# junejunejune/c_orb_slam

Hardware: AMD Instinct MI355X
Metric: tracking FPS + ORB matches/sec, KITTI-00 stereo; local-BA iter/sec (higher is better)
Workload: dtype u8

## Files before the change

### c_orb_slam_amd/_lib.py

```python
import ctypes as C
import os
import re
from pathlib import Path

import numpy as np

PKG = Path(__file__).resolve().parent
ROOT = PKG.parent
LIB_PATH = Path(os.environ["ORBGPU_LIB"]) if os.environ.get("ORBGPU_LIB") else PKG / "liborbslam_gpu.so"
HEADER = ROOT / "include" / "orbslam_gpu.h"

ORB_OK, ORB_E_INVALID, ORB_E_HIP, ORB_E_CAPACITY, ORB_E_NODEVICE = 0, -1, -2, -3, -4
_ERR = {ORB_E_INVALID: "ORB_E_INVALID", ORB_E_HIP: "ORB_E_HIP", ORB_E_CAPACITY: "ORB_E_CAPACITY",
        ORB_E_NODEVICE: "ORB_E_NODEVICE"}

KP_DTYPE = np.dtype([("x", "<f4"), ("y", "<f4"), ("size", "<f4"), ("angle", "<f4"),
                     ("response", "<f4"), ("octave", "<i4"), ("class_id", "<i4")])
assert KP_DTYPE.itemsize == 28


class OrbGpuError(RuntimeError):
    def __init__(self, code, what=""):
        super().__init__(f"{what}: {_ERR.get(code, code)}")
        self.code = code
# ... 181 lines not shown
    L.Optimizer_last_trace.argtypes = [vp, vp, i32, P(i32), vp, vp, i32, P(i32)]
    L.Optimizer_last_timings.argtypes = [vp]
    L.Optimizer_PoseOptimization.argtypes = [P(pose_problem), vp, vp, P(i32)]
    L.Optimizer_PoseOptimization_batch.argtypes = [i32, vp, vp, vp, vp]
    L.Optimizer_PoseOptimization_batch_device.argtypes = [i32, vp, vp, vp, vp]
    L.Optimizer_OptimizeSim3.argtypes = [vp, vp, vp, P(i32)]
    L.Optimizer_OptimizeSim3_batch.argtypes = [i32, vp, vp, vp, vp]
    L.Optimizer_OptimizeEssentialGraph.argtypes = [vp, i32, vp]
    L.Optimizer_PoseOptimization_frames_device.argtypes = [i32, vp, vp, vp, vp]
    L.Optimizer_pose_timing.argtypes = [i32, vp]
    L.orbgpu_unit_ba_struct.argtypes = [i32, i32, i32, vp, vp, vp, vp, vp, vp, i32, vp, C.c_longlong]
    L.Frame_UnprojectStereo_batch_device.argtypes = [vp, i32, vp]
    L.Frame_UndistortKeyPoints.argtypes = [vp, vp]
    L.Frame_UndistortKeyPoints_batch.argtypes = [vp, i32, vp]
    L.Frame_ComputeImageBounds.argtypes = [vp, i32, i32, vp, vp, i32, vp]
    L.Frame_ComputeStereoFromRGBD.argtypes = [vp, vp, vp]
    L.Frame_ComputeStereoFromRGBD_batch.argtypes = [vp, i32, vp, vp]
    L.ORBvocabulary_create.argtypes = [P(vp)]
    L.ORBvocabulary_destroy.argtypes = [vp]
    L.ORBvocabulary_loadFromTextFile.argtypes = [vp, C.c_char_p]
    L.ORBvocabulary_info.argtypes = [vp, vp, vp, vp, vp, vp, vp]
    L.ORBvocabulary_transform.argtypes = [vp, vp, i32, i32, vp]
    L.ORBvocabulary_transform_batch.argtypes = [vp, i32, vp, vp, i32, vp]
    L.ORBvocabulary_transform_features.argtypes = [vp, vp, i32, i32, vp, vp, vp]
    L.ORBvocabulary_score.argtypes = [vp, vp, vp, i32, i32, vp, vp, vp, vp]
    L.orbgpu_unit_ldlt_solve.argtypes = [i32, vp, vp, vp, i32, P(i32)]
    L.orbgpu_unit_csum.argtypes = [vp, i32, vp]
    L.orbgpu_unit_pnp_layout.argtypes = [i32, vp, vp, vp, vp]
    L.MapPoint_CreateStereo_batch_device.argtypes = [vp, i32, vp]
    L.Tracking_PrepareLocalSearch_batch_device.argtypes = [vp, i32, vp]
    L.ORBmatcher_SearchDense_batch.argtypes = [vp, i32, vp, vp, vp, vp, vp, vp, vp]
    L.ORBmatcher_last_dense_timing.argtypes = [vp, vp, vp]
    L.ORBmatcher_SearchLocalPoints_batch.argtypes = [vp, i32, vp, vp, vp, f32, f32, f32, vp, vp]
    L.Frame_isInFrustum_batch.argtypes = [vp, i32, vp, vp, f32, f32, vp, vp, vp, vp, vp, vp, vp]
    L.ORBmatcher_enable_timing.argtypes = [vp, i32]
    L.ORBmatcher_last_timings.argtypes = [vp, vp, vp]
    L.ORBmatcher_last_search_plan.argtypes = [vp, vp]
    L.orbgpu_unit_ldlt_factor.argtypes = [i32, vp, vp]
    L.orbgpu_unit_wave_tree.argtypes = [vp, vp]
    L.orbgpu_unit_shared_div.argtypes = [vp, vp, i32, vp]
    L.orbgpu_unit_set_csum_lds_max.argtypes = [i32]
    L.orbgpu_unit_set_scale_small_max.argtypes = [i32]
    L.orbgpu_unit_set_struct_gpu_min_edges.argtypes = [i32]
    L.orbgpu_unit_set_posegraph_check.argtypes = [i32]
    L.orbgpu_unit_ba_struct_all.argtypes = [i32, i32, i32, vp, vp, vp, vp, vp, vp, i32, i32, vp, C.c_longlong, vp]
    L.orbgpu_unit_nd_order.argtypes = [i32, vp, vp, i32, vp, vp, vp]
    L.orbgpu_unit_sim3.argtypes = [i32, i32, vp, vp, vp, vp]
    L.orbgpu_unit_essgraph_stage.argtypes = [vp, C.c_double, vp]
    L.orbgpu_unit_set_ess_dense_max.argtypes = [i32]
    L.orbgpu_debug_prof.argtypes = [vp]
    L.orbgpu_debug_prof_match.argtypes = [vp]
    L.orbgpu_debug_prof_extract.argtypes = [vp]
    L.orbgpu_debug_extract_plan.argtypes = [vp, vp, vp, vp]
    L.KeyFrameDatabase_create.argtypes = [vp, P(vp)]
    L.KeyFrameDatabase_destroy.argtypes = [vp]
    L.KeyFrameDatabase_add.argtypes = [vp, C.c_int32, vp, vp, i32]
    L.KeyFrameDatabase_add_batch.argtypes = [vp, i32, vp, vp, vp, vp]
    L.KeyFrameDatabase_erase.argtypes = [vp, C.c_int32]
    L.KeyFrameDatabase_clear.argtypes = [vp]
    L.KeyFrameDatabase_size.argtypes = [vp, P(i32), P(C.c_longlong)]
    L.KeyFrameDatabase_set_covisibles.argtypes = [vp, C.c_int32, i32, vp]
    L.KeyFrameDatabase_DetectLoopCandidates.argtypes = [vp, vp, vp]
    L.KeyFrameDatabase_DetectRelocalizationCandidates.argtypes = [vp, vp, vp]
    L.KeyFrameDatabase_DetectRelocalizationCandidates_batch.argtypes = [vp, i32, vp, vp]
    L.KeyFrameDatabase_enable_timing.argtypes = [vp, i32]
    L.KeyFrameDatabase_last_timings.argtypes = [vp, vp]
    L.orbgpu_unit_set_kfdb_initial_capacity.argtypes = [i32, i32]
    L.Map_create.argtypes = [P(vp)]
    L.Map_destroy.argtypes = [vp]
    L.Map_clear.argtypes = [vp]
    L.Map_size.argtypes = [vp, P(i32), P(C.c_longlong), P(C.c_longlong)]
    L.Map_AddKeyFrame.argtypes = [vp, C.c_int32, i32, vp, vp]
    L.Map_SetMapPointMatches.argtypes = [vp, C.c_int32, i32, vp, vp, vp]
    L.Map_EraseMapPoint.argtypes = [vp, C.c_int32]
    L.Map_ReplaceMapPoint.argtypes = [vp, C.c_int32, C.c_int32]
    L.Map_EraseKeyFrame.argtypes = [vp, C.c_int32]
    L.Map_SetNeighbours.argtypes = [vp, C.c_int32, i32, vp, C.c_int32, i32, vp]
    L.KeyFrame_UpdateConnections.argtypes = [vp, C.c_int32, vp]
    L.KeyFrame_UpdateConnections_batch.argtypes = [vp, i32, vp, vp]
    L.Tracking_UpdateLocalMap_batch.argtypes = [vp, vp, i32, vp]
    L.Map_enable_timing.argtypes = [vp, i32]
    L.Map_last_timings.argtypes = [vp, vp]
    L.orbgpu_unit_set_map_initial_capacity.argtypes = [i32, i32, i32]
    L.orbgpu_unit_set_map_chunk.argtypes = [i32]
    L.orbgpu_unit_set_map_lds_slots.argtypes = [i32]
    L.Initializer_create.argtypes = [vp, i32, vp, f32, i32, P(vp)]
    L.Initializer_destroy.argtypes = [vp]
    L.Initializer_Initialize.argtypes = [vp, i32, vp, vp, vp, vp, vp, vp, vp, P(i32), vp]
    L.Initializer_enable_timing.argtypes = [vp, i32]
    L.Initializer_last_timings.argtypes = [vp, vp]
    L.Sim3Solver_create.argtypes = [i32, vp, vp, vp, vp, vp, i32, vp, vp, i32, P(vp)]
    L.Sim3Solver_destroy.argtypes = [vp]
    L.Sim3Solver_set_ransac.argtypes = [vp, C.c_double, i32, i32]
    L.Sim3Solver_iterate.argtypes = [vp, i32, vp, P(i32), vp, P(i32), vp, P(i32)]
    L.Sim3Solver_iterate_batch.argtypes = [i32, vp, i32, vp, vp, vp, vp, vp, vp]
    L.Sim3Solver_get_estimate.argtypes = [vp, vp, vp, vp]
    L.Sim3Solver_get_state.argtypes = [vp, P(i32), P(i32), P(i32)]
    L.Sim3Solver_enable_timing.argtypes = [i32]
    L.Sim3Solver_last_timings.argtypes = [vp, vp]
    _lib = L
    return L


class orb_rng(C.Structure):
    _fields_ = [("tbl", C.c_int32 * 31), ("f", C.c_int32), ("r", C.c_int32)]

# ... 117 lines not shown
```

### c_orb_slam_amd/csrc/capi_extract.cpp

```cpp
#include <new>

#include "capi_handles.hpp"

extern "C" {

int orbgpu_device_available(void) {
    int n = 0;
    if (hipGetDeviceCount(&n) != hipSuccess) return 0;
    return n > 0 ? 1 : 0;
}

const char* orbgpu_version(void) { return "c_orb_slam_amd 0.2 (gfx950)"; }
int orbgpu_abi_version(void) { return ORBGPU_ABI_VERSION; }

int ORBextractor_create(int nfeatures, float scaleFactor, int nlevels, int iniThFAST, int minThFAST,
                        int max_width, int max_height, int max_batch, ORBextractor_h* out) {
    if (!out || nfeatures < 0 || nlevels < 1 || nlevels > 15 || scaleFactor <= 1.0f || max_width <= 0 ||
        max_height <= 0 || max_batch <= 0 || max_batch > 2047)
        return ORB_E_INVALID;
    *out = nullptr;
    auto* ex = new (std::nothrow) orbgpu::Extractor(nfeatures, scaleFactor, nlevels, iniThFAST, minThFAST);
    if (!ex) return ORB_E_INVALID;
    int rc = ex->init_device(max_width, max_height, max_batch);
    if (rc) {
// ... 63 lines not shown
    return rc == 0 ? ORB_OK : (rc == -2 ? ORB_E_HIP : ORB_E_INVALID);
}

int ORBextractor_get_levels(ORBextractor_h h, int* nlevels, float* scaleFactor) {
    if (!h) return ORB_E_INVALID;
    if (nlevels) *nlevels = h->ex->nlevels();
    if (scaleFactor) *scaleFactor = h->ex->scale_factor();
    return ORB_OK;
}

int ORBextractor_get_scale_tables(ORBextractor_h h, float* scale, float* invScale, float* sigma2, float* invSigma2,
                                  int* nFeaturesPerLevel) {
    if (!h) return ORB_E_INVALID;
    const auto* ex = h->ex;
    for (int l = 0; l < ex->nlevels(); l++) {
        if (scale) scale[l] = ex->scale()[l];
        if (invScale) invScale[l] = ex->inv_scale()[l];
        if (sigma2) sigma2[l] = ex->sigma2()[l];
        if (invSigma2) invSigma2[l] = ex->inv_sigma2()[l];
        if (nFeaturesPerLevel) nFeaturesPerLevel[l] = ex->n_per_level()[l];
    }
    return ORB_OK;
}

void* ORBextractor_stream(ORBextractor_h h) { return h ? (void*)h->ex->stream() : nullptr; }

int ORBextractor_reserve_cus(ORBextractor_h h, int one_in_n) {
    if (!h || one_in_n < 0 || one_in_n == 1) return ORB_E_INVALID;
    const int r = h->ex->reserve_cus(one_in_n);
    return r == -4 ? ORB_E_NODEVICE : r == -1 ? ORB_E_INVALID : (r ? ORB_E_HIP : ORB_OK);
}

int ORBextractor_share_stream(ORBextractor_h h, ORBextractor_h with) {
    if (!h || !with) return ORB_E_INVALID;
    const int r = h->ex->share_stream(with->ex);
    return r == -4 ? ORB_E_NODEVICE : (r ? ORB_E_HIP : ORB_OK);
}

int ORBextractor_last_timings(ORBextractor_h h, float* ms6) {
    if (!h || !ms6) return ORB_E_INVALID;
    return h->ex->timings(ms6);
}

int ORBextractor_last_corner_count(ORBextractor_h h, long long* total) {
    if (!h || !total) return ORB_E_INVALID;
    return h->ex->corner_total(total) ? ORB_E_INVALID : ORB_OK;
}

int orbgpu_debug_extract_plan(ORBextractor_h h, int* flags, int* chain_from, int* tile_rows) {
    if (!h) return ORB_E_INVALID;
    return h->ex->last_plan(flags, chain_from, tile_rows) ? ORB_E_INVALID : ORB_OK;
}

}
```

### c_orb_slam_amd/csrc/orb_extract.hip

```cpp
#include "orb_extract.hpp"

#include <algorithm>
#include <atomic>
#include <chrono>
#include <cmath>
#include <cstring>
#include <thread>

namespace orbgpu {

__constant__ int8_t c_pattern[256 * 4];
__constant__ int8_t c_disc[2 * 1024];
__constant__ int c_ndisc;
__constant__ int c_umax[16];
__constant__ int c_gauss[7];

static const int8_t kPattern[256 * 4] = {
#include "brief_pattern.inc"
};

__device__ __forceinline__ int xcd_tile(int bid, int nb) { return (bid & 7) * (nb >> 3) + (bid >> 3); }
static inline unsigned grid8(int n) { return (unsigned)((n + 7) & ~7); }
constexpr int kFastSplitLevel = 3;

// ... 4 lines not shown
    uint4 o;
    if (x0 >= 0 && x0 + 15 < W) {
        const uintptr_t a = (uintptr_t)(srow + x0);
        const uint32_t* a32 = reinterpret_cast<const uint32_t*>(a & ~(uintptr_t)3);
        const uint32_t sh = (uint32_t)(a & 3);
        const uint32_t w0 = a32[0], w1 = a32[1], w2 = a32[2], w3 = a32[3];
        const uint32_t w4 = sh ? a32[4] : 0u;
        o.x = __builtin_amdgcn_alignbyte(w1, w0, sh);
        o.y = __builtin_amdgcn_alignbyte(w2, w1, sh);
        o.z = __builtin_amdgcn_alignbyte(w3, w2, sh);
        o.w = __builtin_amdgcn_alignbyte(w4, w3, sh);
    } else {
        uint32_t v[4] = {0, 0, 0, 0};
#pragma unroll
        for (int k = 0; k < 16; k++) v[k >> 2] |= (uint32_t)srow[refl101(x0 + k, W)] << (8 * (k & 3));
        o = make_uint4(v[0], v[1], v[2], v[3]);
    }
    return o;
}

__global__ void __launch_bounds__(256) k_pyr_level0(const uint8_t* __restrict__ src, size_t src_stride, int step,
                                                    int W, int H, uint8_t* __restrict__ pyr, size_t img_bytes,
                                                    int pitch, int ph, int* __restrict__ zero0,
                                                    int* __restrict__ zero1) {
    const int b = blockIdx.y;
    if (blockIdx.x == 0 && b == 0 && threadIdx.x == 0) {
        *zero0 = 0;
        *zero1 = 0;
    }
    const int chunks = pitch >> 4;
    const int t = blockIdx.x * blockDim.x + threadIdx.x;
    if (t >= chunks * ph) return;
    const int py = t / chunks, px0 = (t - py * chunks) * 16;
    const uint4 o = pyr_l0_chunk(src + (size_t)b * src_stride, step, W, H, py, px0);
    *reinterpret_cast<uint4*>(pyr + (size_t)b * img_bytes + (size_t)py * pitch + px0) = o;
}

constexpr int kPyrTileH[2] = {16, 32};
template <int TH>
constexpr int stage_regs() { return (((TH * 5 + 3) / 4 + 3) * ((PT_W * 5 / 4 + 12) / 4) + 255) / 256; }
typedef unsigned int u32x4v __attribute__((ext_vector_type(4)));
__device__ __forceinline__ __amdgpu_buffer_rsrc_t slab_rsrc(uint8_t* p, size_t bytes) {
    const unsigned long long a = (unsigned long long)p;
    const unsigned lo = __builtin_amdgcn_readfirstlane((unsigned)a);
    const unsigned hi = __builtin_amdgcn_readfirstlane((unsigned)(a >> 32));
    void* q = (void*)(((unsigned long long)hi << 32) | lo);
    return __builtin_amdgcn_make_buffer_rsrc(q, (short)0, (int)bytes, 0x00020000);
}
template <int TH, bool WT>
__device__ __forceinline__ void pyr_tile(uint8_t* __restrict__ base, size_t img_bytes, size_t src_off, int src_pitch,
                                         size_t dst_off, int dst_pitch, int w, int h, const int* __restrict__ xofs,
                                         const short2* __restrict__ xalpha, const int2* __restrict__ yrows,
                                         const short2* __restrict__ ybeta, const PyrTile& tl, uint32_t* s_src) {
    const int lane = threadIdx.x & 63, wid = threadIdx.x >> 6;
    const uint32_t* S32 = reinterpret_cast<const uint32_t*>(base + src_off + (size_t)(kEdge + tl.sr0) * src_pitch + tl.sc0);
    const int spw = src_pitch >> 2;
    {
        const int nw = tl.nsr * tl.nsw;
        for (int t0 = threadIdx.x; t0 < nw; t0 += 256 * stage_regs<TH>()) {
            uint32_t v[stage_regs<TH>()];
#pragma unroll
            for (int u = 0; u < stage_regs<TH>(); u++) {
                const int t = t0 + 256 * u;
                const int r = t / tl.nsw, c = t - r * tl.nsw;
                v[u] = t < nw ? S32[(size_t)r * spw + c] : 0u;
            }
#pragma unroll
            for (int u = 0; u < stage_regs<TH>(); u++)
                if (t0 + 256 * u < nw) s_src[t0 + 256 * u] = v[u];
        }
    }
    const int px = tl.px0 + 4 * lane;
    const bool col_ok = px < dst_pitch;
    int lx[4];
    short2 al[4];
#pragma unroll
    for (int k = 0; k < 4; k++) {
        const int x = refl101(px + k - kEdge, w);
        lx[k] = col_ok ? xofs[x] + kEdge - tl.sc0 : 0;
        al[k] = col_ok ? xalpha[x] : make_short2(0, 0);
    }
    int2 rr[TH / 4];
    short2 bb[TH / 4];
#pragma unroll
    for (int i = 0; i < TH / 4; i++) {
        const int j = wid + 4 * i;
        const int y = refl101(tl.py0 + min(j, tl.nrow - 1) - kEdge, h);
        rr[i] = yrows[y];
        bb[i] = ybeta[y];
    }
    __syncthreads();
    if (!col_ok) return;
    const uint8_t* sb = reinterpret_cast<const uint8_t*>(s_src);
    const int rowb = tl.nsw * 4;
    __amdgpu_buffer_rsrc_t rs;
    if (WT) rs = slab_rsrc(base, img_bytes);
#pragma unroll
    for (int i = 0; i < TH / 4; i++) {
        const int j = wid + 4 * i;
        if (j >= tl.nrow) break;
        const int py = tl.py0 + j;
        const uint8_t* R0 = sb + (rr[i].x - tl.sr0) * rowb;
        const uint8_t* R1 = sb + (rr[i].y - tl.sr0) * rowb;
        const short2 bb_ = bb[i];
        uint32_t v = 0;
#pragma unroll
        for (int k = 0; k < 4; k++) {
            const int sx = lx[k];
            const short2 a = al[k];
            const int D0 = R0[sx] * a.x + R0[sx + (a.y != 0)] * a.y;
            const int D1 = R1[sx] * a.x + R1[sx + (a.y != 0)] * a.y;
            const int o = (((bb_.x * (D0 >> 4)) >> 16) + ((bb_.y * (D1 >> 4)) >> 16) + 2) >> 2;
            v |= (uint32_t)(uint8_t)o << (8 * k);
        }
        if (WT)
            __builtin_amdgcn_raw_buffer_store_b32(v, rs, (int)(dst_off + (size_t)py * dst_pitch + px), 0, 16);
        else
            *reinterpret_cast<uint32_t*>(base + dst_off + (size_t)py * dst_pitch + px) = v;
    }
}

template <int TH>
__global__ void __launch_bounds__(256) k_pyr_resize(uint8_t* __restrict__ pyr, size_t img_bytes, size_t src_off,
                                                    int src_pitch, size_t dst_off, int dst_pitch, int dst_ph, int w,
                                                    int h, const int* __restrict__ xofs,
                                                    const short2* __restrict__ xalpha, const int2* __restrict__ yrows,
                                                    const short2* __restrict__ ybeta,
                                                    const PyrTile* __restrict__ tiles, int ntiles) {
    extern __shared__ uint32_t s_src[];
    const int tile = xcd_tile(blockIdx.x, gridDim.x);
    if (tile >= ntiles) return;
    const PyrTile tl = tiles[tile];
    (void)dst_ph;
    pyr_tile<TH, false>(pyr + (size_t)blockIdx.y * img_bytes, img_bytes, src_off, src_pitch, dst_off, dst_pitch, w, h,
                        xofs, xalpha, yrows, ybeta, tl, s_src);
}

typedef __attribute__((address_space(1))) int g_i32;
__device__ __forceinline__ void flow_publish(int* cnt) {
    asm volatile("s_waitcnt vmcnt(0)" ::: "memory");
    __syncthreads();
    if (threadIdx.x == 0) __hip_atomic_fetch_add((g_i32*)cnt, 1, __ATOMIC_RELAXED, __HIP_MEMORY_SCOPE_AGENT);
}
__device__ __forceinline__ bool flow_wait(int* cnt, int need) {
    for (int spins = 0; __hip_atomic_load((g_i32*)cnt, __ATOMIC_RELAXED, __HIP_MEMORY_SCOPE_AGENT) < need; spins++) {
        if (spins > (1 << 22)) return false;
        __builtin_amdgcn_s_sleep(2);
    }
    return true;
// ... 1117 lines not shown
            for (auto& cp : csel) {
                CellGroup g{};
                const CellDesc& tl = cells_[rowb[rp.first] + cp.first];
                const CellDesc& br = cells_[rowb[rp.first + rp.second - 1] + cp.first + cp.second - 1];
                g.r0 = tl.r0; g.c0 = tl.c0;
                g.rows = br.r1 - tl.r0; g.cols = br.c1 - tl.c0;
                g.rsplit = rp.second == 2 ? tl.r1 - tl.r0 - 6 : std::max(g.rows - 6, 0);
                g.csplit = cp.second == 2 ? tl.c1 - tl.c0 - 6 : std::max(g.cols - 6, 0);
                g.pitch = tl.pitch;
                g.lvl_off = tl.lvl_off;
                for (int k = 0; k < 4; k++) {
                    const int di = k >> 1, dj = k & 1;
                    g.cell[k] = -1;
                    if (di >= rp.second || dj >= cp.second) continue;
                    const int c = rowb[rp.first + di] + cp.first + dj;
                    const CellDesc& cd = cells_[c];
                    g.cell[k] = c;
                    g.cap[k] = cd.cap;
                    g.slot_off[k] = cd.slot_off;
                    g.xadd[k] = cd.offx - (cd.c0 - g.c0);
                    g.yadd[k] = cd.offy - (cd.r0 - g.r0);
                }
                groups_.push_back(g);
            }
    }
    if (groups_.size() > 65535) return -1;
    tiles_.clear();
    for (int l = 0; l < nlevels_; l++) {
        const LevelHost& L = levels_[l];
        for (int ty = 0; ty < (L.h + BT_H - 1) / BT_H; ty++)
            for (int tx = 0; tx < (L.w + BT_W - 1) / BT_W; tx++) {
                BlurTile t;
                t.off = L.off; t.pitch = L.pitch; t.w = L.w; t.h = L.h; t.tx = tx; t.ty = ty;
                t.boff = L.boff; t.bpitch = L.bpitch;
                tiles_.push_back(t);
            }
    }
    std::vector<uint8_t> tabs;
    auto push = [&tabs](const void* p, size_t n) -> size_t {
        size_t o = (tabs.size() + 15) & ~(size_t)15;
        tabs.resize(o + n);
        memcpy(tabs.data() + o, p, n);
        return o;
    };
    tab_off_.assign(nlevels_, {0, 0, 0, 0});
    std::vector<std::vector<int>> yrAll(nlevels_);
    xofsAll_.assign(nlevels_, {});
    xalAll_.assign(nlevels_, {});
    ptiles_.clear();
    ptile_begin_.assign(2 * (nlevels_ + 1), 0);
    ptile_n_.assign(2 * nlevels_, 0);
    plds_.assign(2 * nlevels_, 0);
    ptile_th_.assign(2 * nlevels_, 0);
    for (int l = 1; l < nlevels_; l++) {
        const int sw = levels_[l - 1].w, sh = levels_[l - 1].h, dw = levels_[l].w, dh = levels_[l].h;
        const double scale_x = 1. / ((double)dw / sw), scale_y = 1. / ((double)dh / sh);
        std::vector<int> xofs(dw);
        std::vector<short> xal(2 * dw);
        int xmax = dw;
        auto sat_s = [](float v) { long i = std::lrint(v); return (short)std::min(32767L, std::max(-32768L, i)); };
        for (int dx = 0; dx < dw; dx++) {
            float fx = (float)((dx + 0.5) * scale_x - 0.5);
            int sx = (int)std::floor(fx);
            fx -= sx;
            if (sx < 0) { fx = 0; sx = 0; }
            if (sx + 1 >= sw) {
                xmax = std::min(xmax, dx);
                if (sx >= sw - 1) { fx = 0; sx = sw - 1; }
            }
            xofs[dx] = sx;
            xal[2 * dx] = sat_s((1.f - fx) * 2048);
            xal[2 * dx + 1] = sat_s(fx * 2048);
        }
        for (int dx = xmax; dx < dw; dx++) { xal[2 * dx] = 2048; xal[2 * dx + 1] = 0; }
        std::vector<int> yr(2 * dh);
        std::vector<short> yb(2 * dh);
        for (int dy = 0; dy < dh; dy++) {
            float fy = (float)((dy + 0.5) * scale_y - 0.5);
            int sy = (int)std::floor(fy);
            fy -= sy;
            yr[2 * dy] = std::min(std::max(sy, 0), sh - 1);
            yr[2 * dy + 1] = std::min(std::max(sy + 1, 0), sh - 1);
            yb[2 * dy] = sat_s((1.f - fy) * 2048);
            yb[2 * dy + 1] = sat_s(fy * 2048);
        }
        {
            const LevelHost& D = levels_[l];
            auto refl = [](int p, int len) {
                if (len == 1) return 0;
                while (p < 0 || p >= len) p = p < 0 ? -p : 2 * len - p - 2;
                return p;
            };
          for (int v = 0; v < 2; v++) {
            ptile_begin_[v * (nlevels_ + 1) + l] = (int)ptiles_.size();
            auto make = [&](int py0, int px0, int nrow, PyrTile& t) {
                int r0 = 1 << 30, r1 = -1, c0 = 1 << 30, c1 = -1;
                for (int py = py0; py < std::min(py0 + nrow, D.ph); py++) {
                    const int y = refl(py - kEdge, dh);
                    r0 = std::min(r0, yr[2 * y]);
                    r1 = std::max(r1, yr[2 * y + 1]);
                }
                for (int px = px0; px < std::min(px0 + PT_W, D.pitch); px++) {
                    const int x = refl(px - kEdge, dw);
                    c0 = std::min(c0, xofs[x]);
                    c1 = std::max(c1, xofs[x] + 1);
                }
                t.py0 = py0; t.px0 = px0; t.nrow = std::min(nrow, D.ph - py0);
                t.sr0 = r0; t.nsr = r1 - r0 + 1;
                t.sc0 = (c0 + kEdge) & ~3;
                t.nsw = (c1 + kEdge - t.sc0) / 4 + 1;
                return (size_t)t.nsr * t.nsw * 4 <= (size_t)kPyrLdsMax;
            };
            int nrow = kPyrTileH[v];
            for (bool ok = false; !ok;) {
                ok = true;
                for (int py0 = 0; py0 < D.ph && ok; py0 += nrow)
                    for (int px0 = 0; px0 < D.pitch && ok; px0 += PT_W) {
                        PyrTile t;
                        ok = make(py0, px0, nrow, t);
                    }
                if (!ok && --nrow < 1) return -1;
            }
            size_t lds = 0;
            for (int py0 = 0; py0 < D.ph; py0 += nrow)
                for (int px0 = 0; px0 < D.pitch; px0 += PT_W) {
                    PyrTile t;
                    make(py0, px0, nrow, t);
                    if ((size_t)(t.sc0 + 4 * t.nsw) > (size_t)levels_[l - 1].pitch) return -1;
                    lds = std::max(lds, (size_t)t.nsr * t.nsw * 4);
                    ptiles_.push_back(t);
                }
            plds_[v * nlevels_ + l] = (int)lds;
            ptile_th_[v * nlevels_ + l] = nrow;
            ptile_n_[v * nlevels_ + l] = (int)ptiles_.size() - ptile_begin_[v * (nlevels_ + 1) + l];
          }
        }
        yrAll[l] = yr;
        xofsAll_[l] = xofs;
        xalAll_[l] = xal;
        tab_off_[l][0] = push(xofs.data(), xofs.size() * 4);
        tab_off_[l][1] = push(xal.data(), xal.size() * 2);
        tab_off_[l][2] = push(yr.data(), yr.size() * 4);
        tab_off_[l][3] = push(yb.data(), yb.size() * 2);
    }
    if (plan_chain(yrAll)) return -1;
    auto F = [](void*& p) { if (p) (void)hipFree(p); p = nullptr; };
    F(d_pyr_); F(d_blur_); F(d_slots_); F(d_counts_); F(d_cells_); F(d_tiles_); F(d_lcb_); F(d_work_); F(d_groups_);
    F(d_cellslot_);
    work_B_ = -1;
    F(d_packed_); F(d_hdr_); F(d_sel_); F(d_levels_); F(d_tabs_); F(d_ptiles_);
    const int B = maxB_;
    if (d_chain_) (void)hipFree(d_chain_);
    d_chain_ = nullptr;
    if (chain_) {
        ORB_HIP_CHECK(hipMalloc(&d_chain_, chainTab_.size()));
        ORB_HIP_CHECK(hipMemcpy(d_chain_, chainTab_.data(), chainTab_.size(), hipMemcpyHostToDevice));
    }
    ORB_HIP_CHECK(hipMalloc(&d_ptiles_, std::max<size_t>(ptiles_.size(), 1) * sizeof(PyrTile)));
    if (!ptiles_.empty())
        ORB_HIP_CHECK(hipMemcpy(d_ptiles_, ptiles_.data(), ptiles_.size() * sizeof(PyrTile), hipMemcpyHostToDevice));
    if (d_flowcnt_) (void)hipFree(d_flowcnt_);
    d_flowcnt_ = nullptr;
    for (int v = 0; v < 2; v++) {
        ptile_th_[v * nlevels_] = kPyrTileH[v];
        int nb = 0, lds = 0;
        for (int l = 0; l < nlevels_; l++) {
            nb += (levels_[l].ph + ptile_th_[v * nlevels_ + l] - 1) / ptile_th_[v * nlevels_ + l];
            lds = std::max(lds, plds_[v * nlevels_ + l]);
        }
        flowBands_[v] = nb;
        flowLds_[v] = lds;
    }
    ORB_HIP_CHECK(hipMalloc(&d_flowcnt_, (size_t)std::max(flowBands_[0], flowBands_[1]) * B * 4));
    ORB_HIP_CHECK(hipMalloc(&d_pyr_, img_bytes_ * B));
    ORB_HIP_CHECK(hipMalloc(&d_blur_, blur_bytes_ * B));
    ORB_HIP_CHECK(hipMemset(d_blur_, 0, blur_bytes_ * B));
    ORB_HIP_CHECK(hipMalloc(&d_slots_, slots_per_image_ * 4 * B));
    ORB_HIP_CHECK(hipMalloc(&d_counts_, cells_.size() * 4 * B));
    ORB_HIP_CHECK(hipMalloc(&d_cells_, cells_.size() * sizeof(CellDesc)));
    ORB_HIP_CHECK(hipMemcpy(d_cells_, cells_.data(), cells_.size() * sizeof(CellDesc), hipMemcpyHostToDevice));
    ORB_HIP_CHECK(hipMalloc(&d_groups_, groups_.size() * sizeof(CellGroup)));
    ORB_HIP_CHECK(hipMemcpy(d_groups_, groups_.data(), groups_.size() * sizeof(CellGroup), hipMemcpyHostToDevice));
// ... 47 lines not shown
    ORB_HIP_CHECK(hipMemcpy(d_octlv_, ol.data(), ol.size() * sizeof(OctLevelDev), hipMemcpyHostToDevice));
    ORB_HIP_CHECK(hipMalloc(&d_jobsel_, (size_t)B * nlevels_ * jcap_ * 4));
    ORB_HIP_CHECK(hipMalloc(&d_jobcnt_, (size_t)B * nlevels_ * 4));
    ORB_HIP_CHECK(hipMalloc(&d_gscr_, (size_t)packed_cap_ * 3 * 2));
    ORB_HIP_CHECK(hipMalloc(&d_nout_, (size_t)(B + 1) * 4));
    ORB_HIP_CHECK(hipFree(d_sel_));
    d_sel_ = nullptr;
    sel_cap_ = selcap_ * B;
    ORB_HIP_CHECK(hipMalloc(&d_sel_, (size_t)sel_cap_ * sizeof(int2)));
    if (h_nout_) (void)hipHostFree(h_nout_);
    ORB_HIP_CHECK(hipHostMalloc((void**)&h_nout_, (size_t)(B + 1) * 4));
    geomW_ = W;
    geomH_ = H;
    return 0;
}

int Extractor::extract(const uint8_t* imgs, int B, int W, int H, int step, size_t img_stride,
                       bool imgs_on_device, orb_kp* kps, uint8_t* desc, int cap, bool out_on_device,
                       int* n_out, const uint8_t* const* list) {
    if (B <= 0 || B > maxB_ || W <= 0 || H <= 0) return -1;
    if (W > maxW_ || H > maxH_) return -1;
    if (int e = setup_geometry(W, H)) return e;
    hipStream_t s = stream_;
    const uint8_t* src = imgs;
    if (!imgs_on_device) {
        const size_t need = img_stride * (B - 1) + (size_t)step * (H - 1) + W;
        if (need > in_cap_) {
            if (d_in_) (void)hipFree(d_in_);
            ORB_HIP_CHECK(hipMalloc(&d_in_, need));
            in_cap_ = need;
        }
        if (h_in_) ORB_HIP_CHECK(hipEventSynchronize(ev_[0]));
        if (need > h_in_cap_) {
            if (h_in_) (void)hipHostFree(h_in_);
            h_in_ = nullptr;
            h_in_cap_ = 0;
            ORB_HIP_CHECK(hipHostMalloc(&h_in_, need));
            h_in_cap_ = need;
        }
        if (list) {
            const size_t one = (size_t)step * (H - 1) + W;
            for (int b = 0; b < B; b++) std::memcpy((uint8_t*)h_in_ + img_stride * b, list[b], one);
        } else {
            std::memcpy(h_in_, imgs, need);
        }
        ORB_HIP_CHECK(hipMemcpyAsync(d_in_, h_in_, need, hipMemcpyHostToDevice, s));
        src = (const uint8_t*)d_in_;
    }
    ORB_HIP_CHECK(hipEventRecord(ev_[0], s));
    const int ncells = (int)cells_.size();
    if (work_B_ != B && build_work(B)) return -2;
    const bool split = fastSplit_ && work_part_[0] > 0 && work_part_[1] > 0;
    int planFlags = (split ? kPlanFastSplit : 0) | (evBlur_ ? kPlanBlurSide : 0) | (B >= 8 ? kPlanTile32 : 0);
    int planChainFrom = 0;
    {
        const LevelHost& L0 = levels_[0];
        const int n = (L0.pitch / 16) * L0.ph;
        const bool flow = flow_ && !split && !chain_;
        if (flow) {
            const int v = B >= 8 ? 1 : 0;
            ORB_HIP_CHECK(hipMemsetAsync(d_flowcnt_, 0, (size_t)flowBands_[v] * B * 4, s));
            const FlowArgs A = flow_args(v, B);
            int tasks = 0;
            for (int l = 0; l < nlevels_; l++) tasks += B * A.L[l].ntiles;
            auto kern = v ? k_pyr_flow<kPyrTileH[1]> : k_pyr_flow<kPyrTileH[0]>;
            hipLaunchKernelGGL(kern, dim3(tasks), dim3(256), flowLds_[v], s, src, img_stride, step, W, H,
                               (uint8_t*)d_pyr_, img_bytes_, A, (const PyrTile*)d_ptiles_, (const uint8_t*)d_tabs_,
                               d_flowcnt_, 1, d_gtotal_, (int*)d_nout_ + B);
        } else {
            hipLaunchKernelGGL(k_pyr_level0, dim3((n + 255) / 256, B), dim3(256), 0, s, src, img_stride, step, W, H,
                               (uint8_t*)d_pyr_, img_bytes_, L0.pitch, L0.ph, d_gtotal_, (int*)d_nout_ + B);
        }
        const int lend = flow ? 1 : chain_ && !split ? chainFrom_ : nlevels_;
        if (flow) planFlags |= kPlanFlow;
        if (!flow && lend < nlevels_) {
            planFlags |= kPlanChain;
            planChainFrom = lend;
        }
        for (int l = 1; l < lend; l++) {
            if (split && l == kFastSplitLevel) {
                ORB_HIP_CHECK(hipEventRecord(evPyrA_, s));
                ORB_HIP_CHECK(hipStreamWaitEvent(side_, evPyrA_, 0));
                hipLaunchKernelGGL(k_fast_cells, dim3(work_part_[0]), dim3(256), 0, side_, (const uint8_t*)d_pyr_,
                                   img_bytes_, (const CellGroup*)d_groups_, iniTh_, minTh_, (uint32_t*)d_slots_,
                                   slots_per_image_, (int*)d_counts_, ncells, (const int*)d_work_);
                ORB_HIP_CHECK(hipEventRecord(evFastA_, side_));
            }
            const LevelHost& L = levels_[l];
            const LevelHost& P = levels_[l - 1];
            const uint8_t* T = (const uint8_t*)d_tabs_;
            const int v = B >= 8 ? 1 : 0, pb = v * (nlevels_ + 1) + l;
            const int nt = ptile_n_[v * nlevels_ + l];
            auto kern = v ? k_pyr_resize<kPyrTileH[1]> : k_pyr_resize<kPyrTileH[0]>;
            hipLaunchKernelGGL(kern, dim3(grid8(nt), B), dim3(256), plds_[v * nlevels_ + l], s, (uint8_t*)d_pyr_, img_bytes_,
                               P.off, P.pitch, L.off, L.pitch, L.ph, L.w, L.h,
                               (const int*)(T + tab_off_[l][0]), (const short2*)(T + tab_off_[l][1]),
                               (const int2*)(T + tab_off_[l][2]), (const short2*)(T + tab_off_[l][3]),
                               (const PyrTile*)d_ptiles_ + ptile_begin_[pb], nt);
        }
        if (!flow && lend < nlevels_) {
            const uint8_t* T = (const uint8_t*)d_chain_;
            const LevelHost& P = levels_[lend - 1];
            hipLaunchKernelGGL(k_pyr_chain, dim3(chainK_, B), dim3(256), chainLds_, s, (uint8_t*)d_pyr_, img_bytes_,
                               (long long)P.off, P.pitch, P.w, (const ChainLevel*)T, nlevels_ - lend,
                               (const int4*)(T + chainStripOff_), (const uint16_t*)(T + chainRowOff_),
                               (const uint8_t*)d_tabs_, chainSrcLds_, chainSrcRp_);
        }
    }
    ORB_HIP_CHECK(hipGetLastError());
    ORB_HIP_CHECK(hipEventRecord(ev_[1], s));
    static const bool blurEarly = [] {
        const char* e = getenv("ORBGPU_BLUR_EARLY");
        return e && e[0] == '1';
    }();
    if (blurEarly && !evBlur_) {
        planFlags |= kPlanBlurEarly;
        hipLaunchKernelGGL(k_blur7, dim3(grid8((int)tiles_.size()), B), dim3(256), 0, s, (const uint8_t*)d_pyr_,
                           (uint8_t*)d_blur_, img_bytes_, blur_bytes_, (const BlurTile*)d_tiles_, (int)tiles_.size());
    }
    if (evBlur_) {
        ORB_HIP_CHECK(hipStreamWaitEvent(side_, ev_[1], 0));
        hipLaunchKernelGGL(k_blur7, dim3(grid8((int)tiles_.size()), B), dim3(256), 0, side_, (const uint8_t*)d_pyr_,
                           (uint8_t*)d_blur_, img_bytes_, blur_bytes_, (const BlurTile*)d_tiles_, (int)tiles_.size());
        ORB_HIP_CHECK(hipEventRecord(evBlur_, side_));
    }
    if (split) {
// ... 15 lines not shown
    if (int e = octree_launch(oin, B, nlevels_, (const OctLevelDev*)d_octlv_, (uint32_t*)d_jobsel_, (int*)d_jobcnt_,
                              jcap_, (uint16_t*)d_gscr_, (size_t)packed_cap_, cap, (int2*)d_sel_, selcap_,
                              (int*)d_nout_, d_err, s))
        return e;
    ORB_HIP_CHECK(hipEventRecord(ev_[5], s));
    if (evBlur_)
        ORB_HIP_CHECK(hipStreamWaitEvent(s, evBlur_, 0));
    else if (!blurEarly)
        hipLaunchKernelGGL(k_blur7, dim3(grid8((int)tiles_.size()), B), dim3(256), 0, s, (const uint8_t*)d_pyr_,
                           (uint8_t*)d_blur_, img_bytes_, blur_bytes_, (const BlurTile*)d_tiles_, (int)tiles_.size());
    ORB_HIP_CHECK(hipEventRecord(ev_[2], s));
    orb_kp_dev* okps = (orb_kp_dev*)kps;
    uint8_t* odesc = desc;
    if (!out_on_device) {
        const size_t nk = (size_t)B * cap;
        if (nk > out_cap_) {
            if (d_kps_) (void)hipFree(d_kps_);
            if (d_desc_) (void)hipFree(d_desc_);
            ORB_HIP_CHECK(hipMalloc(&d_kps_, nk * sizeof(orb_kp_dev)));
            ORB_HIP_CHECK(hipMalloc(&d_desc_, nk * 32));
            out_cap_ = nk;
        }
        okps = (orb_kp_dev*)d_kps_;
        odesc = (uint8_t*)d_desc_;
    }
    {
        const int gx = (selcap_ + 3) / 4;
        const int nwg = B >= 8 ? gx * 8 * ((B + 7) / 8) : gx * B;
        hipLaunchKernelGGL(k_orient_desc, dim3(nwg), dim3(256), 0, s, (const uint8_t*)d_pyr_,
                           (const uint8_t*)d_blur_, img_bytes_, blur_bytes_, (const int2*)d_sel_, selcap_,
                           (const int*)d_nout_, levelArgs_, okps, odesc, cap, gx, B);
    }
    ORB_HIP_CHECK(hipGetLastError());
    ORB_HIP_CHECK(hipMemcpyAsync(h_nout_, d_nout_, (size_t)(B + 1) * 4, hipMemcpyDeviceToHost, s));
    ORB_HIP_CHECK(hipEventRecord(ev_[6], s));
    ORB_HIP_CHECK(stream_wait(s));
    const int err = h_nout_[B];
    for (int b = 0; b < B; b++) n_out[b] = h_nout_[b];
    if (err & 1) return -3;
    if (err) return -1;
    if (!out_on_device) {
        for (int b = 0; b < B; b++) {
            if (n_out[b] == 0) continue;
            ORB_HIP_CHECK(hipMemcpyAsync(kps + (size_t)b * cap, okps + (size_t)b * cap, (size_t)n_out[b] * sizeof(orb_kp_dev),
                                         hipMemcpyDeviceToHost, s));
            ORB_HIP_CHECK(hipMemcpyAsync(desc + (size_t)b * cap * 32, odesc + (size_t)b * cap * 32, (size_t)n_out[b] * 32,
                                         hipMemcpyDeviceToHost, s));
        }
        ORB_HIP_CHECK(stream_wait(s));
    }
    last_B_ = B;
    planFlags_ = planFlags;
    planChainFrom_ = planChainFrom;
    return 0;
}

int Extractor::last_plan(int* flags, int* chain_from, int* tile_rows) const {
    if (last_B_ <= 0) return -1;
    if (flags) *flags = planFlags_;
    if (chain_from) *chain_from = planChainFrom_;
    if (tile_rows)
        for (int i = 0; i < 2 * nlevels_; i++) tile_rows[i] = ptile_th_[i];
    return 0;
}

int Extractor::corner_total(long long* total) {
    if (last_B_ <= 0 || !d_gtotal_) return -1;
    int v = 0;
    ORB_HIP_CHECK(hipStreamSynchronize(stream_));
    ORB_HIP_CHECK(hipMemcpy(&v, d_gtotal_, 4, hipMemcpyDeviceToHost));
    *total = v;
    return 0;
}

int Extractor::get_blurred(int index, int level, uint8_t* dst, int dst_step, int* w, int* h) {
    if (level < 0 || level >= nlevels_ || index < 0 || index >= last_B_ || !d_blur_) return -1;
    const LevelHost& L = levels_[level];
    *w = L.w;
    *h = L.h;
    if (!dst) return 0;
    ORB_HIP_CHECK(hipMemcpy2D(dst, dst_step, (const uint8_t*)d_blur_ + (size_t)index * blur_bytes_ + L.boff, L.bpitch,
                              L.w, L.h, hipMemcpyDeviceToHost));
    return 0;
}

int debug_prof_extract(unsigned long long* out32) {
#ifdef ORBGPU_PROF
    ORB_HIP_CHECK(hipMemcpyFromSymbol(out32, HIP_SYMBOL(g_orbgpu_prof), sizeof(unsigned long long) * 16));
    unsigned long long z[32] = {};
    ORB_HIP_CHECK(hipMemcpyToSymbol(HIP_SYMBOL(g_orbgpu_prof), z, sizeof(z)));
    return octree_prof_read(out32 + 16);
#else
    (void)out32;
    return -1;
#endif
}

int Extractor::timings(float* ms6) {
    float t[6] = {0};
    (void)hipEventElapsedTime(&t[0], ev_[0], ev_[1]);
    (void)hipEventElapsedTime(&t[1], ev_[5], ev_[2]);
    (void)hipEventElapsedTime(&t[2], ev_[1], ev_[3]);
    (void)hipEventElapsedTime(&t[3], ev_[3], ev_[4]);
    (void)hipEventElapsedTime(&t[4], ev_[4], ev_[5]);
    (void)hipEventElapsedTime(&t[5], ev_[2], ev_[6]);
    for (int i = 0; i < 6; i++) ms6[i] = t[i];
// ... 16 lines not shown
```

### c_orb_slam_amd/csrc/orb_extract.hpp

```cpp
#pragma once
#include <atomic>
#include <condition_variable>
#include <cstddef>
#include <cstdint>
#include <mutex>
#include <thread>
#include <vector>
#include <array>

#include "orb_common.hpp"
#include "octree.hpp"
#include "../../include/orbslam_gpu.h"

namespace orbgpu {

struct orb_kp_dev {
    float x, y, size, angle, response;
    int32_t octave, class_id;
};
static_assert(sizeof(orb_kp_dev) == 28, "cv::KeyPoint layout");

struct CellDesc {
    int r0, r1, c0, c1;
    int offx, offy;
    int pitch, cap, slot_off, level;
    long long lvl_off;
};

struct CellGroup {
    int r0, c0, rows, cols;
    int rsplit, csplit;
    int pitch, pad;
    long long lvl_off;
    int cell[4], cap[4], slot_off[4];
    int xadd[4], yadd[4];
};

struct BlurTile {
    long long off, boff;
    int pitch, bpitch, w, h, tx, ty;
};

constexpr int PT_W = 256, kPyrLdsMax = 48 * 1024;
struct PyrTile {
    int py0, px0, nrow, sr0, nsr, sc0, nsw, pad;
};

struct ChainLevel {
    long long off;
    int w, h, pitch, rp, lds, xofs, xal, yr, yb, nph;
};
constexpr int kChainLdsMax = 64 * 1024;

struct FlowLevel {
    long long off;
    int pitch, ph, w, h;
    int task0, ntiles;
    int tile0;
    int band0, th, ncol;
    int xofs, xal, yr, yb;
};
struct FlowArgs {
    FlowLevel L[16];
    int nl, nbands;
};

struct LevelDev {
    long long off, boff;
    int pitch, bpitch;
    float scale, kp_size;
};
constexpr int kMaxLevels = 16;
struct LevelArgs {
    LevelDev lv[kMaxLevels];
};

constexpr int kPlanFlow = 1, kPlanChain = 2, kPlanFastSplit = 4, kPlanBlurSide = 8, kPlanBlurEarly = 16,
              kPlanTile32 = 32;

struct LevelHost {
    int w, h, pw, ph, pitch, bpitch;
    size_t off, boff;
};

class Extractor {
public:
    Extractor(int nfeatures, float scaleFactor, int nlevels, int iniTh, int minTh);
    ~Extractor();
    int init_device(int maxW, int maxH, int maxBatch);
    int extract(const uint8_t* imgs, int B, int W, int H, int step, size_t img_stride, bool imgs_on_device,
                orb_kp* kps, uint8_t* desc, int cap, bool out_on_device, int* n_out,
                const uint8_t* const* list = nullptr);
    int cvt_color(const uint8_t* src, int B, int W, int H, int channels, int rgb, int step, size_t img_stride,
                  bool src_on_device, uint8_t* gray, int gray_step, size_t gray_stride);
    int get_level(int index, int level, uint8_t* dst, int dst_step, int* w, int* h);
    int get_blurred(int index, int level, uint8_t* dst, int dst_step, int* w, int* h);
    int timings(float* ms6);
    int corner_total(long long* total);
    int last_plan(int* flags, int* chain_from, int* tile_rows) const;
    hipStream_t stream() const { return stream_; }
    int reserve_cus(int one_in_n);
    int share_stream(Extractor* with);
    int build_work(int B);
    const uint8_t* pyramid_base() const { return (const uint8_t*)d_pyr_; }
    size_t pyramid_image_bytes() const { return img_bytes_; }
    const std::vector<LevelHost>& levels() const { return levels_; }
    int last_batch() const { return last_B_; }

    int nlevels() const { return nlevels_; }
    float scale_factor() const { return scaleFactor_; }
    const std::vector<float>& scale() const { return scale_; }
    const std::vector<float>& inv_scale() const { return invScale_; }
    const std::vector<float>& sigma2() const { return sigma2_; }
    const std::vector<float>& inv_sigma2() const { return invSigma2_; }
    const std::vector<int>& n_per_level() const { return nPerLevel_; }

private:
    static void gaussian_taps(int taps[7]);
    int setup_geometry(int W, int H);
    void release();

    int nfeatures_;
    double scaleFactorD_;
    float scaleFactor_;
    int nlevels_, iniTh_, minTh_;
    std::vector<float> scale_, invScale_, sigma2_, invSigma2_;
    std::vector<int> nPerLevel_, umax_;

    int maxW_ = 0, maxH_ = 0, maxB_ = 0;
    int geomW_ = -1, geomH_ = -1;
    std::vector<LevelHost> levels_;
    LevelArgs levelArgs_{};
    std::vector<CellDesc> cells_;
    std::vector<CellGroup> groups_;
    std::vector<int> level_cell_begin_;
    std::vector<BlurTile> tiles_;
    std::vector<PyrTile> ptiles_;
    std::vector<int> ptile_begin_, ptile_n_, plds_;
    std::vector<int> ptile_th_;
    bool flow_ = false;
    int* d_flowcnt_ = nullptr;
    int flowBands_[2] = {0, 0}, flowLds_[2] = {0, 0};
    FlowArgs flow_args(int v, int B) const;
    int plan_chain(const std::vector<std::vector<int>>& yr);
    bool chain_ = false;
    int chainK_ = 0, chainLds_ = 0, chainFrom_ = 0, chainSrcLds_ = 0, chainSrcRp_ = 0;
    std::vector<std::vector<int>> xofsAll_;
    std::vector<std::vector<short>> xalAll_;
    size_t chainStripOff_ = 0, chainRowOff_ = 0;
    std::vector<uint8_t> chainTab_;
    void* d_chain_ = nullptr;
    void* d_cellslot_ = nullptr;
    std::vector<std::array<size_t, 4>> tab_off_;
    size_t img_bytes_ = 0, blur_bytes_ = 0, slots_per_image_ = 0;
    int packed_cap_ = 0, sel_cap_ = 0;
    int last_B_ = 0;
    int planFlags_ = 0, planChainFrom_ = 0;

    hipStream_t stream_ = nullptr;
    bool ownStream_ = true;
    int lent_ = 0;
    hipEvent_t ev_[7] = {};
    hipStream_t side_ = nullptr;
    hipEvent_t evBlur_ = nullptr;
    bool fastSplit_ = false;
    hipEvent_t evPyrA_ = nullptr, evFastA_ = nullptr;
    void *d_in_ = nullptr, *d_pyr_ = nullptr, *d_blur_ = nullptr, *d_slots_ = nullptr, *d_counts_ = nullptr;
    void *d_ptiles_ = nullptr;
    void *d_cells_ = nullptr, *d_tiles_ = nullptr, *d_lcb_ = nullptr, *d_packed_ = nullptr, *d_hdr_ = nullptr;
    void *d_sel_ = nullptr, *d_levels_ = nullptr, *d_tabs_ = nullptr, *d_kps_ = nullptr, *d_desc_ = nullptr;
    int* d_gtotal_ = nullptr;
    void* d_work_ = nullptr;
    void* d_groups_ = nullptr;
    int work_B_ = -1, work_n_ = 0;
    int work_part_[2] = {0, 0};
    bool d_gtotal_alias_ = false;
    size_t in_cap_ = 0, out_cap_ = 0;
    void* h_in_ = nullptr;
    size_t h_in_cap_ = 0;
    void *d_jobsel_ = nullptr, *d_jobcnt_ = nullptr, *d_octlv_ = nullptr, *d_gscr_ = nullptr, *d_nout_ = nullptr;
    int jcap_ = 0, selcap_ = 0;
    int* h_nout_ = nullptr;

};

int debug_prof_extract(unsigned long long* out32);

}
```

### include/orbslam_gpu.h

```cpp
#ifndef ORBSLAM_GPU_H
#define ORBSLAM_GPU_H
#include <stdbool.h>
#include <stdint.h>
#include <stddef.h>

#ifdef __cplusplus
extern "C" {
#endif

#define ORB_OK 0
#define ORB_E_INVALID -1
#define ORB_E_HIP -2
#define ORB_E_CAPACITY -3
#define ORB_E_NODEVICE -4

typedef struct orb_kp {
    float x, y, size, angle, response;
    int32_t octave, class_id;
} orb_kp;

int orbgpu_device_available(void);
const char* orbgpu_version(void);
#define ORBGPU_ABI_VERSION 2
int orbgpu_abi_version(void);
// ... 594 lines not shown
                                       int bRobust, const volatile bool* stop, ba_result* R);

int Optimizer_last_trace(double* solve_ini_chi2, double* solve_chi2, int solve_cap, int* n_solves,
                         double* trial_chi2, double* trial_lambda, int trial_cap, int* n_trials);
int Optimizer_last_timings(double* ms2);

int orbgpu_unit_ldlt_solve(int n, const double* S, const double* b, double* x, int variant, int* ok);
int orbgpu_unit_csum(const double* v, int n, double* out);
int orbgpu_unit_ldlt_factor(int n, const double* S, double* out);
int orbgpu_unit_pnp_layout(int n, const int* N, const int* K, const int* minSet, long long* out4);
int orbgpu_unit_ba_struct(int nkf, int npt, int ne, const int32_t* edge_kf, const int32_t* edge_pt,
                          const uint8_t* edge_level, const uint8_t* kf_fixed, const int32_t* kf_id,
                          const int32_t* pt_id, int level, int32_t* out, long long cap);
int orbgpu_unit_ba_struct_all(int nkf, int npt, int ne, const int32_t* edge_kf, const int32_t* edge_pt,
                              const uint8_t* edge_level, const uint8_t* kf_fixed, const int32_t* kf_id,
                              const int32_t* pt_id, int level, int gpu, int32_t* out, long long cap,
                              long long* n_out);
int orbgpu_unit_wave_tree(const double* v64, double* out);
int orbgpu_unit_shared_div(const double* a, const double* b, int n, double* out);
int orbgpu_unit_set_csum_lds_max(int m2_max);
int orbgpu_unit_set_scale_small_max(int terms);
int orbgpu_unit_set_struct_gpu_min_edges(int edges);
int orbgpu_unit_set_posegraph_check(int on);
int orbgpu_unit_nd_order(int n, const int32_t* adjStart, const int32_t* adj, int leaf, int32_t* perm,
                         int32_t* n_nodes, int32_t* height);
int orbgpu_unit_sim3(int op, int n, const double* a, const double* b, const double* c, double* out);
typedef struct essgraph_stage {
    int solver;
    int nV;
    int ok;
    int32_t* sysIdx;
    double* meas;
    double* err;
    double* chi2e;
    double* J;
    double* H;
    double* b;
    double* x_solve;
    double* x;
    double* est_trial;
    double* chi2e_trial;
    double chi2, chi2_trial, scale;
} essgraph_stage;
int orbgpu_unit_essgraph_stage(const essgraph_problem* P, double lambda, essgraph_stage* out);
int orbgpu_unit_set_ess_dense_max(int rows);
int orbgpu_unit_set_kfdb_initial_capacity(int slots, int entries);
int orbgpu_unit_set_map_initial_capacity(int slots, int cells, int points);
int orbgpu_unit_set_map_chunk(int frames);
int orbgpu_unit_set_map_lds_slots(int slots);
int orbgpu_debug_prof(unsigned long long* out32);
int orbgpu_debug_prof_match(unsigned long long* out32);
int orbgpu_debug_prof_extract(unsigned long long* out32);
int orbgpu_debug_extract_plan(ORBextractor_h h, int* flags, int* chain_from, int* tile_rows);

#ifdef __cplusplus
}
#endif
#endif
```

Baseline: 44140.

## Add packed-row pyramid resize path using byte-permute and udot2 taps

Adds a packed path to the pyramid bilinear resize kernel for levels where consecutive output rows share source rows and four output columns fit in an 8-byte source window. In that path each wave handles contiguous output rows, caches horizontal passes for reused source rows, and computes taps with alignbyte/perm plus udot2. The LDS staging loop also drops the per-element divide by stepping offsets incrementally, and the wave index is made scalar. Adds LDS slack, an env opt-out, and a debug query for which levels took the packed path.

```diff
diff --git a/c_orb_slam_amd/_lib.py b/c_orb_slam_amd/_lib.py
--- a/c_orb_slam_amd/_lib.py
+++ b/c_orb_slam_amd/_lib.py
@@ -257,6 +257,7 @@
     L.orbgpu_debug_prof_match.argtypes = [vp]
     L.orbgpu_debug_prof_extract.argtypes = [vp]
     L.orbgpu_debug_extract_plan.argtypes = [vp, vp, vp, vp]
+    L.orbgpu_debug_pyramid_packed_levels.argtypes = [vp, vp]
     L.KeyFrameDatabase_create.argtypes = [vp, P(vp)]
     L.KeyFrameDatabase_destroy.argtypes = [vp]
     L.KeyFrameDatabase_add.argtypes = [vp, C.c_int32, vp, vp, i32]
diff --git a/c_orb_slam_amd/csrc/capi_extract.cpp b/c_orb_slam_amd/csrc/capi_extract.cpp
--- a/c_orb_slam_amd/csrc/capi_extract.cpp
+++ b/c_orb_slam_amd/csrc/capi_extract.cpp
@@ -139,4 +139,9 @@
     return h->ex->last_plan(flags, chain_from, tile_rows) ? ORB_E_INVALID : ORB_OK;
 }
 
+int orbgpu_debug_pyramid_packed_levels(ORBextractor_h h, int* mask) {
+    if (!h || !mask) return ORB_E_INVALID;
+    return h->ex->last_pyr_packed(mask) ? ORB_E_INVALID : ORB_OK;
 }
+
+}
diff --git a/c_orb_slam_amd/csrc/orb_extract.hip b/c_orb_slam_amd/csrc/orb_extract.hip
--- a/c_orb_slam_amd/csrc/orb_extract.hip
+++ b/c_orb_slam_amd/csrc/orb_extract.hip
@@ -80,18 +80,26 @@
                                          size_t dst_off, int dst_pitch, int w, int h, const int* __restrict__ xofs,
                                          const short2* __restrict__ xalpha, const int2* __restrict__ yrows,
                                          const short2* __restrict__ ybeta, const PyrTile& tl, uint32_t* s_src) {
-    const int lane = threadIdx.x & 63, wid = threadIdx.x >> 6;
+    const int lane = threadIdx.x & 63, wid = __builtin_amdgcn_readfirstlane(threadIdx.x >> 6);
     const uint32_t* S32 = reinterpret_cast<const uint32_t*>(base + src_off + (size_t)(kEdge + tl.sr0) * src_pitch + tl.sc0);
     const int spw = src_pitch >> 2;
     {
         const int nw = tl.nsr * tl.nsw;
+        const uint32_t nsw = (uint32_t)tl.nsw, dcol = 256u % nsw;
+        const uint32_t dbytes = ((256u / nsw) * (uint32_t)spw + dcol) * 4u, dwrap = ((uint32_t)spw - nsw) * 4u;
+        uint32_t c = threadIdx.x % nsw, boff = ((threadIdx.x / nsw) * (uint32_t)spw + c) * 4u;
+        const uint8_t* S8 = reinterpret_cast<const uint8_t*>(S32);
         for (int t0 = threadIdx.x; t0 < nw; t0 += 256 * stage_regs<TH>()) {
             uint32_t v[stage_regs<TH>()];
 #pragma unroll
             for (int u = 0; u < stage_regs<TH>(); u++) {
-                const int t = t0 + 256 * u;
-                const int r = t / tl.nsw, c = t - r * tl.nsw;
-                v[u] = t < nw ? S32[(size_t)r * spw + c] : 0u;
+                v[u] = t0 + 256 * u < nw ? *reinterpret_cast<const uint32_t*>(S8 + boff) : 0u;
+                c += dcol;
+                boff += dbytes;
+                if (c >= nsw) {
+                    c -= nsw;
+                    boff += dwrap;
+                }
             }
 #pragma unroll
             for (int u = 0; u < stage_regs<TH>(); u++)
@@ -108,11 +116,12 @@
         lx[k] = col_ok ? xofs[x] + kEdge - tl.sc0 : 0;
         al[k] = col_ok ? xalpha[x] : make_short2(0, 0);
     }
+    const bool packed = tl.packed != 0;
     int2 rr[TH / 4];
     short2 bb[TH / 4];
 #pragma unroll
     for (int i = 0; i < TH / 4; i++) {
-        const int j = wid + 4 * i;
+        const int j = packed ? wid * (TH / 4) + i : wid + 4 * i;
         const int y = refl101(tl.py0 + min(j, tl.nrow - 1) - kEdge, h);
         rr[i] = yrows[y];
         bb[i] = ybeta[y];
@@ -123,6 +132,56 @@
     const int rowb = tl.nsw * 4;
     __amdgpu_buffer_rsrc_t rs;
     if (WT) rs = slab_rsrc(base, img_bytes);
+    if (packed) {
+        if (wid * (TH / 4) >= tl.nrow) return;
+        const int mn = min(min(lx[0], lx[1]), min(lx[2], lx[3]));
+        const uint32_t sh = (uint32_t)mn & 3u;
+        const uint8_t* wbase = sb + (mn & ~3);
+        typedef unsigned short u16x2 __attribute__((ext_vector_type(2)));
+        uint32_t sel[4];
+        u16x2 aw[4];
+#pragma unroll
+        for (int k = 0; k < 4; k++) {
+            const uint32_t o = (uint32_t)(lx[k] - mn);
+            sel[k] = 0x0c000c00u | o | ((o + 1) << 16);
+            aw[k] = u16x2{(unsigned short)al[k].x, (unsigned short)al[k].y};
+        }
+        auto hpass = [&](int r, uint32_t (&d)[4]) {
+            const uint32_t* p = reinterpret_cast<const uint32_t*>(wbase + (r - tl.sr0) * rowb);
+            const uint32_t w0 = p[0], w1 = p[1], w2 = p[2];
+            const uint32_t x0 = __builtin_amdgcn_alignbyte(w1, w0, sh), x1 = __builtin_amdgcn_alignbyte(w2, w1, sh);
+#pragma unroll
+            for (int k = 0; k < 4; k++) {
+                const uint32_t pp = __builtin_amdgcn_perm(x1, x0, sel[k]);
+                d[k] = __builtin_amdgcn_udot2(__builtin_bit_cast(u16x2, pp), aw[k], 0u, false) >> 4;
+            }
+        };
+        int kp = -1, kq = -1;
+        uint32_t dp[4], dq[4];
+        const uint32_t doff = (uint32_t)dst_off + (uint32_t)px;
+#pragma unroll
+        for (int i = 0; i < TH / 4; i++) {
+            const int r0 = rr[i].x, r1 = rr[i].y;
+            const bool cross = (r0 == kq || r1 == kp) && r0 != kp && r1 != kq;
+            const int rp = cross ? r1 : r0, rq = cross ? r0 : r1;
+            const uint32_t bp = (uint32_t)(cross ? bb[i].y : bb[i].x), bq = (uint32_t)(cross ? bb[i].x : bb[i].y);
+            if (rp != kp) hpass(rp, dp);
+            if (rq != kq) hpass(rq, dq);
+            kp = rp;
+            kq = rq;
+            uint32_t o[4];
+#pragma unroll
+            for (int k = 0; k < 4; k++) o[k] = ((__umul24(bp, dp[k]) >> 16) + (__umul24(bq, dq[k]) >> 16) + 2) >> 2;
+            const uint32_t v = __builtin_amdgcn_perm(__builtin_amdgcn_perm(o[3], o[2], 0x0c0c0400u),
+                                                     __builtin_amdgcn_perm(o[1], o[0], 0x0c0c0400u), 0x05040100u);
+            const int py = tl.py0 + min(wid * (TH / 4) + i, tl.nrow - 1);
+            if (WT)
+                __builtin_amdgcn_raw_buffer_store_b32(v, rs, (int)(doff + (uint32_t)(py * dst_pitch)), 0, 16);
+            else
+                *reinterpret_cast<uint32_t*>(base + (doff + (uint32_t)(py * dst_pitch))) = v;
+        }
+        return;
+    }
 #pragma unroll
     for (int i = 0; i < TH / 4; i++) {
         const int j = wid + 4 * i;
@@ -1346,6 +1405,7 @@
     ptile_n_.assign(2 * nlevels_, 0);
     plds_.assign(2 * nlevels_, 0);
     ptile_th_.assign(2 * nlevels_, 0);
+    pyrPacked_.assign(nlevels_, 0);
     for (int l = 1; l < nlevels_; l++) {
         const int sw = levels_[l - 1].w, sh = levels_[l - 1].h, dw = levels_[l].w, dh = levels_[l].h;
         const double scale_x = 1. / ((double)dw / sw), scale_y = 1. / ((double)dh / sh);
@@ -1385,6 +1445,24 @@
                 while (p < 0 || p >= len) p = p < 0 ? -p : 2 * len - p - 2;
                 return p;
             };
+            static const bool byteTaps = [] {
+                const char* e = getenv("ORBGPU_PYR_BYTE_TAPS");
+                return e && e[0] == '1';
+            }();
+            bool shares = false;
+            for (int dy = 0; dy + 1 < dh && !shares; dy++) shares = yr[2 * (dy + 1)] <= yr[2 * dy + 1];
+            bool fits = !byteTaps && shares && (size_t)dw * dh <= (size_t)kPyrPackedMaxPx;
+            for (int px0 = 0; px0 < D.pitch && fits; px0 += 4) {
+                int lo = 1 << 30, hi = -1;
+                for (int k = 0; k < 4; k++) {
+                    const int x = refl(px0 + k - kEdge, dw);
+                    lo = std::min(lo, xofs[x]);
+                    hi = std::max(hi, xofs[x] + 1);
+                }
+                fits = hi - lo + 1 <= 8;
+            }
+            pyrPacked_[l] = fits;
+            const size_t slack = fits ? kPyrLdsSlack : 0;
           for (int v = 0; v < 2; v++) {
             ptile_begin_[v * (nlevels_ + 1) + l] = (int)ptiles_.size();
             auto make = [&](int py0, int px0, int nrow, PyrTile& t) {
@@ -1403,7 +1481,8 @@
                 t.sr0 = r0; t.nsr = r1 - r0 + 1;
                 t.sc0 = (c0 + kEdge) & ~3;
                 t.nsw = (c1 + kEdge - t.sc0) / 4 + 1;
-                return (size_t)t.nsr * t.nsw * 4 <= (size_t)kPyrLdsMax;
+                t.packed = fits;
+                return (size_t)t.nsr * t.nsw * 4 + slack <= (size_t)kPyrLdsMax;
             };
             int nrow = kPyrTileH[v];
             for (bool ok = false; !ok;) {
@@ -1421,7 +1500,7 @@
                     PyrTile t;
                     make(py0, px0, nrow, t);
                     if ((size_t)(t.sc0 + 4 * t.nsw) > (size_t)levels_[l - 1].pitch) return -1;
-                    lds = std::max(lds, (size_t)t.nsr * t.nsw * 4);
+                    lds = std::max(lds, (size_t)t.nsr * t.nsw * 4 + slack);
                     ptiles_.push_back(t);
                 }
             plds_[v * nlevels_ + l] = (int)lds;
@@ -1575,7 +1654,7 @@
     if (work_B_ != B && build_work(B)) return -2;
     const bool split = fastSplit_ && work_part_[0] > 0 && work_part_[1] > 0;
     int planFlags = (split ? kPlanFastSplit : 0) | (evBlur_ ? kPlanBlurSide : 0) | (B >= 8 ? kPlanTile32 : 0);
-    int planChainFrom = 0;
+    int planChainFrom = 0, planPacked = 0;
     {
         const LevelHost& L0 = levels_[0];
         const int n = (L0.pitch / 16) * L0.ph;
@@ -1595,6 +1674,7 @@
                                (uint8_t*)d_pyr_, img_bytes_, L0.pitch, L0.ph, d_gtotal_, (int*)d_nout_ + B);
         }
         const int lend = flow ? 1 : chain_ && !split ? chainFrom_ : nlevels_;
+        for (int l = 1; l < (flow ? nlevels_ : lend); l++) planPacked |= pyrPacked_[l] ? 1 << l : 0;
         if (flow) planFlags |= kPlanFlow;
         if (!flow && lend < nlevels_) {
             planFlags |= kPlanChain;
@@ -1716,6 +1796,13 @@
     last_B_ = B;
     planFlags_ = planFlags;
     planChainFrom_ = planChainFrom;
+    planPacked_ = planPacked;
+    return 0;
+}
+
+int Extractor::last_pyr_packed(int* mask) const {
+    if (last_B_ <= 0) return -1;
+    *mask = planPacked_;
     return 0;
 }
 
diff --git a/c_orb_slam_amd/csrc/orb_extract.hpp b/c_orb_slam_amd/csrc/orb_extract.hpp
--- a/c_orb_slam_amd/csrc/orb_extract.hpp
+++ b/c_orb_slam_amd/csrc/orb_extract.hpp
@@ -41,9 +41,9 @@
     int pitch, bpitch, w, h, tx, ty;
 };
 
-constexpr int PT_W = 256, kPyrLdsMax = 48 * 1024;
+constexpr int PT_W = 256, kPyrLdsMax = 48 * 1024, kPyrLdsSlack = 8, kPyrPackedMaxPx = 128 * 1024;
 struct PyrTile {
-    int py0, px0, nrow, sr0, nsr, sc0, nsw, pad;
+    int py0, px0, nrow, sr0, nsr, sc0, nsw, packed;
 };
 
 struct ChainLevel {
@@ -98,6 +98,7 @@
     int timings(float* ms6);
     int corner_total(long long* total);
     int last_plan(int* flags, int* chain_from, int* tile_rows) const;
+    int last_pyr_packed(int* mask) const;
     hipStream_t stream() const { return stream_; }
     int reserve_cus(int one_in_n);
     int share_stream(Extractor* with);
@@ -138,6 +139,7 @@
     std::vector<PyrTile> ptiles_;
     std::vector<int> ptile_begin_, ptile_n_, plds_;
     std::vector<int> ptile_th_;
+    std::vector<char> pyrPacked_;
     bool flow_ = false;
     int* d_flowcnt_ = nullptr;
     int flowBands_[2] = {0, 0}, flowLds_[2] = {0, 0};
@@ -155,7 +157,7 @@
     size_t img_bytes_ = 0, blur_bytes_ = 0, slots_per_image_ = 0;
     int packed_cap_ = 0, sel_cap_ = 0;
     int last_B_ = 0;
-    int planFlags_ = 0, planChainFrom_ = 0;
+    int planFlags_ = 0, planChainFrom_ = 0, planPacked_ = 0;
 
     hipStream_t stream_ = nullptr;
     bool ownStream_ = true;
diff --git a/include/orbslam_gpu.h b/include/orbslam_gpu.h
--- a/include/orbslam_gpu.h
+++ b/include/orbslam_gpu.h
@@ -670,6 +670,7 @@
 int orbgpu_debug_prof_match(unsigned long long* out32);
 int orbgpu_debug_prof_extract(unsigned long long* out32);
 int orbgpu_debug_extract_plan(ORBextractor_h h, int* flags, int* chain_from, int* tile_rows);
+int orbgpu_debug_pyramid_packed_levels(ORBextractor_h h, int* mask);
 
 #ifdef __cplusplus
 }
```

Result: no change. 43730 (-0.9%).
